# Illumina/manta

Hardware: AMD Instinct MI355X
Metric: candidate SV loci assembled+aligned per second (whole node) (higher is better)
Workload: dtype int32; 1 GPU; BASELINE config[1]: synthetic small-indel loci, 80 reads/locus x150bp, k=31..76 step 5, assemble + 10-mer trim + GlobalLargeIndelAligner(2,-8,-24,-1,-1;-100) on 1800 bp windows; loci_per_gpu=10000, reads_per_locus=80, block_loci=10000, workers_per_gpu=1, parallelism=loci sharded over 1 rank(s); per rank a cost-ordered block queue, queue=rank, dist_world=1, mix=False

## Files before the change

### manta_amd/csrc/asm_contig.hpp

```cpp
#pragma once
#ifdef MANTA_WAVE_EMU
#include <set>
#endif
#include "asm_lds.hpp"

namespace manta_dev {

#ifndef MANTA_CK_FAST_CAP
#define MANTA_CK_FAST_CAP 3
#endif
static const unsigned CK_FAST_CAP = MANTA_CK_FAST_CAP;
static const unsigned CK_MAX_EXT = 1020;

struct CkWsLayout {
  uint64_t lane_seq, lane_bits, lane_meta, lane_log, total;
};
static const unsigned CK_SEQ_WORDS = CK_MAX_EXT / 16 + 2;
static const unsigned CK_LOG_QW    = (CK_MAX_EXT + 4) / 4;
WV_HD CkWsLayout ckWorkspaceLayout(const unsigned setw = 2)
{
  CkWsLayout L;
  uint64_t   o = 0;
  L.lane_seq  = asmPut(o, 64ull * 2 * 4 * CK_SEQ_WORDS);
  L.lane_bits = asmPut(o, 64ull * 2 * setw * 8);
// ... 1037 lines not shown
      for (unsigned q = 0; q < SW; ++q) {
        sup.w[q] = lb[q];
        rej.w[q] = lb[SW + q];
      }
      const int32_t* m   = lane_meta + candSlotV * 8;
      nLeft              = unsigned(m[0]);
      nRight             = unsigned(m[1]);
      consB              = m[2];
      consE              = m[3];
      myLen              = nLeft + k + nRight;
    }
    Set      used = setZero();
    bool     aliveL     = lane < nCand;
    unsigned finalCount = 0;
    uint64_t chosen     = 0;
    uint64_t chosenHi   = 0;
    Set normalS;
    for (unsigned q = 0; q < SW; ++q) {
      const unsigned lo = 64 * q;
      normalS.w[q]      = (nNormal >= lo + 64) ? ~uint64_t(0) : ((nNormal > lo) ? ((uint64_t(1) << (nNormal - lo)) - 1) : uint64_t(0));
    }
    while (finalCount < P.opt.maxAssemblyCount) {
      if (!wv::any(aliveL)) break;
      const unsigned usedNormal = popSet(setAnd(used, normalS));
      if (nNormal - usedNormal < P.opt.minUnusedReads) break;
      const Set      fresh  = setAndNot(sup, used);
      const unsigned nFresh = popSet(fresh);
      if (aliveL && popSet(setAnd(fresh, normalS)) < P.opt.minSupportReads) aliveL = false;
      uint64_t key = aliveL ? ((uint64_t(nFresh) << 40) | (uint64_t(myLen) << 8) | uint64_t(63u - lane)) : 0;
      for (int off = 1; off < 64; off <<= 1) {
        const uint64_t o = wv::shfl(key, wv::lane() ^ off);
        key              = (o > key) ? o : key;
      }
      if ((key >> 40) == 0) break;
      const int selected = wv::first(int(63u - unsigned(key & 63u)));
      if (finalCount < 10)
        chosen |= uint64_t(selected) << (6 * finalCount);
      else
        chosenHi |= uint64_t(selected) << (6 * (finalCount - 10));
      if (int(lane) == selected) aliveL = false;
      for (unsigned q = 0; q < SW; ++q) used.w[q] |= wv::readlane(sup.w[q], selected);
      finalCount++;
    }
    auto chosenAt = [&](const unsigned f) { return unsigned(((f < 10) ? (chosen >> (6 * f)) : (chosenHi >> (6 * (f - 10)))) & 63u); };

    AsmLocusOut out;
    out.status            = ASM_OK;
    out.n_contigs         = finalCount;
    out.n_words           = W;
    const unsigned nP     = st ? wv::first(st->nPseudo) : 0u;
    out.n_pseudo          = nP;
    out.final_word_length = k;
    out.n_iterations      = nIter;
    out.cyclic_iterations = cycIters;
    out.reserved          = 0;
    uint64_t seqBytes = 0;
    for (unsigned f = 0; f < finalCount; ++f) seqBytes += wv::readlane(myLen, int(chosenAt(f)));
    const unsigned pLen = (lane < nP) ? unsigned(st->len[lane]) : 0u;
    {
      unsigned t = pLen;
      for (int off = 1; off < 64; off <<= 1) t += wv::shfl(t, wv::lane() ^ off);
      seqBytes += t;
    }
    const uint64_t     bitsWords = uint64_t(finalCount) * 2 * W + nP;
    unsigned long long seqBase = 0, bitsBase = 0;
    if (lane == 0) {
      seqBase  = wv::atomic_add(P.seq_used, (unsigned long long)seqBytes);
      bitsBase = wv::atomic_add(P.bits_used, (unsigned long long)bitsWords);
    }
    seqBase  = wv::readlane(uint64_t(seqBase), 0);
    bitsBase = wv::readlane(uint64_t(bitsBase), 0);
    if (seqBase + seqBytes > P.seq_cap || bitsBase + bitsWords > P.bits_cap) {
      out.status         = ASM_E_OUT_CAPACITY;
      out.n_contigs      = 0;
      out.pseudo_off     = 0;
      out.pseudo_len_off = 0;
      if (lane == 0) P.loci[locus] = out;
      return;
    }
    uint64_t        so = seqBase, bo = bitsBase;
    const uint16_t* gp = gPb();
    for (unsigned f = 0; f < finalCount; ++f) {
      const int      c   = int(chosenAt(f));
      const unsigned sl  = wv::readlane(candSlotV, c);
      const unsigned nL  = wv::readlane(nLeft, c), nR = wv::readlane(nRight, c), len = nL + k + nR;
      const unsigned seedPb = gp[slotNode[sl]];
      for (unsigned i = lane; i < len; i += 64) P.seq_arena[so + i] = uint8_t("ACGT"[contigCode(sl, nL, seedPb, i)]);
      {
        const unsigned half = lane / W, w = lane % W;
        uint64_t       mine = 0;
        for (unsigned q = 0; q < SW; ++q) {
          const uint64_t sq = wv::readlane(sup.w[q], c), rq = wv::readlane(rej.w[q], c);
          if (w == q) mine = half ? rq : sq;
        }
        if (lane < 2 * W) P.bits_arena[bo + lane] = mine;
      }
      const int cb = wv::readlane(consB, c), ce = wv::readlane(consE, c);
      if (lane == 0) {
        AsmContigOut o;
        o.seq_off    = so;
        o.bits_off   = bo;
        o.seq_len    = len;
        o.cons_begin = cb;
        o.cons_end   = int(len) - ce;
        o.reserved   = 0;
        P.contigs[size_t(locus) * P.opt.maxAssemblyCount + f] = o;
      }
      so += len;
      bo += 2 * W;
    }
    out.pseudo_off     = so;
    out.pseudo_len_off = bo;
    if (nP) {
      const uint32_t* pc = G.parena + st->off;
      unsigned        cw = 0;
      for (unsigned p = 0; p < nP; ++p) {
        const unsigned len = wv::readlane(pLen, int(p));
        for (unsigned i = lane; i < len; i += 64) P.seq_arena[so + i] = uint8_t("ACGT"[(pc[cw + (i >> 4)] >> (30 - 2 * (i & 15))) & 3u]);
        if (lane == 0) P.bits_arena[bo + p] = len;
        so += len;
        cw += (len + 15) / 16 + 1;
      }
    }
    if (lane == 0) P.loci[locus] = out;
    if (!C::BIG && G.sched && shareBytes) scheduleEpilogue(locus, seqBase, finalCount, myLen, chosen, chosenHi);
  }

  WV_DEV void scheduleEpilogue(const unsigned locus, const uint64_t seqBase, const unsigned finalCount, const unsigned myLen, const uint64_t chosen,
                               const uint64_t chosenHi)
  {
    const ScheduleParams& S = *G.sched;
    auto lenAt = [&](const unsigned f) { return wv::readlane(myLen, int(((f < 10) ? (chosen >> (6 * f)) : (chosenHi >> (6 * (f - 10)))) & 63u)); };
    if (shareBytes <= SCHED_TABLE_BYTES + 16) return;
    const unsigned lseqBytes = (shareBytes - SCHED_TABLE_BYTES) & ~15u;
    const uint64_t ro0 = wv::readlane(uint64_t(S.ref_off[locus]), 0), ro1 = wv::readlane(uint64_t(S.ref_off[locus + 1]), 0);
    if (ro1 < ro0 || ro1 - ro0 > lseqBytes) return;
    const unsigned refSize = unsigned(ro1 - ro0);
    bool           fits    = true;
    for (unsigned f = 0; f < finalCount; ++f) {
      const unsigned len = lenAt(f);
      if (!schedTableFitsLds(len) || schedStagedBytes(len, refSize) > lseqBytes) fits = false;
    }
    if (!fits) return;
    wv::sync();
    uint32_t* const ltable = reinterpret_cast<uint32_t*>(lds);
    uint8_t* const  lseq   = reinterpret_cast<uint8_t*>(lds) + SCHED_TABLE_BYTES;
    const unsigned  maxAsm = S.max_assembly_count, total = S.n_loci * maxAsm;
    if (lane >= finalCount && lane < maxAsm) {
      SmallSvTaskInfo none = {0, 0, 0, -1};
      S.info[locus * maxAsm + lane] = none;
    }
    uint64_t so  = seqBase;
    unsigned cig = 0;
    for (unsigned f = 0; f < finalCount; ++f) {
      const unsigned        len  = lenAt(f);
      const unsigned        slot = locus * maxAsm + f;
      const SmallSvTaskInfo info = scheduleContig<false>(S, slot, locus, so, len, ltable, lseq, lseqBytes, nullptr);
      wv::sync();
      const int bucket = wv::first(info.bucket);
      if (lane == 0) {
        S.info[slot] = info;
        if (bucket >= 0) {
          const unsigned b       = unsigned(bucket);
          const unsigned winLen  = refSize - unsigned(info.adj_leading_cut) - unsigned(info.adj_trailing_cut);
          const unsigned slabLen = schedSlabLen(S, b, len, winLen);
          S.bucket_ids[size_t(b) * total + wv::atomic_add(&S.bucket_count[b], 1u)] = slot;
          if (wv::atomic_load(&S.bucket_maxref[b]) < slabLen) wv::atomic_max(&S.bucket_maxref[b], slabLen);
        }
      }
      if (bucket >= 0) cig += 4 * len + 16;
      so += len;
      wv::sync();
    }
    if (lane == 0) {
      S.marks[locus] = 1;
      wv::atomic_add(S.n_marked, 1ull);
      if (cig) wv::atomic_add(S.cigar_used, (unsigned long long)cig);
    }
  }

  WV_DEV int run(const unsigned locus)
  {
    tMark = wv::clock();
#ifdef MANTA_WAVE_EMU
#define CK_TRACE(why) do { if (std::getenv("MANTA_EMU_PUNT_TRACE") && lane == 0) std::fprintf(stderr, "  contig_kernel punts locus %u: %s (%u words, %u with a set, k %u)\n", locus, why, nNodes, nFat, k); } while (0)
#else
#define CK_TRACE(why) do { } while (0)
#endif
    if (!load(locus)) {
      CK_TRACE("does not fit this launch's LDS");
      if (C::BIG && lane == 0 && G.stats) wv::atomic_add(&G.stats[7], 1u);
      return CK_PUNT;
    }
    tick(4);
    if (!acyclic && !cyclic && graphHasCycle()) {
      CK_TRACE("cyclic graph");
      return CK_PUNT;
    }
    tick(3);
    loadPool();
    tick(4);
    anyRep = false;
    if ((C::BIG ? contigRoundsStretch() : contigRounds()) != 0) {
      CK_TRACE("contig too long");
      if (C::BIG && lane == 0 && G.stats) wv::atomic_add(&G.stats[7], 1u);
      return CK_PUNT;
    }
    const bool rounds = C::BIG && G.iter != nullptr;
    if (anyRep && !rounds) {
      CK_TRACE("repeat hit");
      return CK_PUNT;
    }
    const unsigned round    = rounds ? G.round : 0u;
    const unsigned nIter    = round + 1;
    const unsigned cycIters = ((round > 0) ? wv::first(G.iter[locus].cyclicIters) : 0u) + (cyclic ? 1u : 0u);
    const LgIter*  st       = (round > 0) ? &G.iter[locus] : nullptr;
    if (anyRep) {
      if (!writePseudo(locus)) {
        CK_TRACE("pseudo arena full");
        if (lane == 0 && G.stats) wv::atomic_add(&G.stats[8], 1u);
        return CK_PUNT;
      }
      st                   = &G.iter[locus];
      const unsigned maxWL = P.locus_max_wl ? P.locus_max_wl[locus] : P.opt.maxWordLength;
      if (k + P.opt.wordStepSize <= maxWL) {
        if (round >= G.last_round) {
          CK_TRACE("more word lengths than rounds");
          if (lane == 0 && G.stats) wv::atomic_add(&G.stats[9], 1u);
          return CK_PUNT;
        }
        if (lane == 0) {
          LgIter* w      = &G.iter[locus];
          w->k           = k + P.opt.wordStepSize;
          w->nIter       = nIter;
          w->cyclicIters = cycIters;
          G.next_ids[wv::atomic_add(G.next_count, 1u)] = locus;
        }
        LG_STAT(7, 1);
        return CK_NEXT;
      }
    }
    selectAndEmit(locus, st, nIter, cycIters);
    tick(7);
    LG_STAT(0, 1);
    LG_STAT(3, nCand);
    LG_STAT(6, acyclic ? 1u : 0u);
    return CK_DONE;
  }
};

template <class C>
WV_DEV void contigKernelBody(const LgArgs& A)
{
  const AsmParams& P = A.P;
  const LgParams&  G = A.G;
  uint8_t*        ws    = G.cws + uint64_t(wv::block_single()) * G.cws_stride;
  char*           lds   = wv::lds_single();
  const unsigned  nLoci = wv::first(wv::atomic_load(&G.class_count[G.cls]));
  const uint32_t* ids   = G.class_ids + size_t(G.cls) * G.class_stride;
  while (true) {
    unsigned slot = 0;
    if (wv::lane() == 0) slot = wv::atomic_add(P.counter, 1u);
    slot = wv::first(slot);
    if (slot >= nLoci) break;
    const unsigned locus = ids[slot];
    LdsContig<C>   c(P, G, lds, ws);
    c.shareBytes = P.lds_bytes;
    const int      rc = c.run(locus);
    wv::sync();
    if (rc == CK_PUNT && wv::lane() == 0) P.punt_ids[wv::atomic_add(P.punt_count, 1u)] = locus;
    wv::sync();
  }
}
#if !MANTA_TU_DEFINES(MANTA_TU_CONTIG)
WV_KERNEL_SINGLE WV_WAVES_PER_SIMD(2) void contig_kernel(const LgArgs A);
#else
WV_KERNEL_SINGLE WV_WAVES_PER_SIMD(2) void contig_kernel(const LgArgs A)
{
  contigKernelBody<LgS>(A);
}
#endif

static const unsigned CK_POOL_WAVES = 12;
static const unsigned CK_POOL_BYTES = 163840;
static const unsigned CK_POOL_HDR   = 64;
static_assert(4 * (1 + CK_POOL_WAVES) <= CK_POOL_HDR && (CK_POOL_BYTES - CK_POOL_HDR) / 16 < 65536, "pool header");

WV_DEV unsigned ckPoolTake(char* pool, const unsigned w, const unsigned units, uint32_t* stat)
{
  uint32_t*      lock  = reinterpret_cast<uint32_t*>(pool);
  uint32_t*      share = lock + 1;
  const unsigned lane  = unsigned(wv::lane());
  const unsigned capU  = (CK_POOL_BYTES - CK_POOL_HDR) / 16;
  unsigned       polls = 0;
  while (true) {
    ++polls;
    unsigned got = 0;
    if (lane == 0) got = (wv::atomic_cas(lock, 0u, 1u) == 0u) ? 1u : 0u;
    if (wv::first(got)) {
      wv::fence_wg();
      unsigned s = 0;
      if (lane >= 1 && lane <= CK_POOL_WAVES) s = wv::atomic_load(&share[lane - 1]) >> 16;
      bool ok = lane <= CK_POOL_WAVES && s + units <= capU;
      for (unsigned v = 0; v < CK_POOL_WAVES; ++v) {
        const unsigned e = wv::atomic_load(&share[v]), a = e & 0xffffu, b = e >> 16;
        if (a < b && s < b && a < s + units) ok = false;
      }
      const uint64_t m  = wv::ballot(ok);
      const unsigned at = m ? wv::readlane(s, wv::ctz(m)) : 0u;
      if (m && lane == 0) wv::atomic_store(&share[w], at | ((at + units) << 16));
// ... 91 lines not shown
```

### manta_amd/csrc/pipeline_kernels.hpp

```cpp
#pragma once
#include "align_kernels.hpp"
#include "assemble_kernels.hpp"
#include "smallsv_trim.hpp"

namespace manta_dev {

WV_DEV SmallSvTaskInfo scheduleSlot(const ScheduleParams& P, const unsigned slot, uint32_t* ltable, uint32_t* gtable)
{
  const unsigned    locus = slot / P.max_assembly_count, ci = slot % P.max_assembly_count;
  const AsmLocusOut lo    = P.loci[locus];
  if (lo.status != ASM_OK || ci >= lo.n_contigs) {
    SmallSvTaskInfo none = {(lo.status != ASM_OK) ? 1 : 0, 0, 0, -1};
    return none;
  }
  const AsmContigOut co = P.contigs[slot];
  return scheduleContig<true>(P, slot, locus, co.seq_off, co.seq_len, ltable, reinterpret_cast<uint8_t*>(ltable) + SCHED_TABLE_BYTES, SCHED_SEQ_BYTES, gtable);
}

static const unsigned SCHED_PEND = 8;
struct SchedPending {
  uint32_t count[16];
  uint32_t maxref[16];
  uint32_t slot[16][SCHED_PEND];
  uint32_t cigarWords;
};
WV_DEV void schedFlush(const ScheduleParams& P, SchedPending* pend, const unsigned bucket, const unsigned total)
{
  const unsigned n = pend->count[bucket];
  if (n == 0) return;
  unsigned pos = 0;
  if (wv::lane() == 0) {
    pos = wv::atomic_add(&P.bucket_count[bucket], n);
    unsigned cur = wv::atomic_load(&P.bucket_maxref[bucket]);
    const unsigned want = pend->maxref[bucket];
    while (cur < want) {
      const unsigned old = wv::atomic_cas(&P.bucket_maxref[bucket], cur, want);
      if (old == cur) break;
      cur = old;
    }
  }
  pos = wv::first(pos);
  if (unsigned(wv::lane()) < n) P.bucket_ids[size_t(bucket) * total + pos + unsigned(wv::lane())] = pend->slot[bucket][wv::lane()];
  wv::sync();
  if (wv::lane() == 0) {
    pend->count[bucket]  = 0;
    pend->maxref[bucket] = 0;
  }
  wv::sync();
}

#if !MANTA_TU_DEFINES(MANTA_TU_GLUE)
WV_KERNEL void smallsv_schedule_kernel(const ScheduleParams P);
#else
WV_KERNEL void smallsv_schedule_kernel(const ScheduleParams P)
{
  const unsigned lane   = unsigned(wv::lane());
  uint32_t*      gtable = P.table_ws + size_t(wv::block()) * P.table_cap;
  uint32_t*      ltable = reinterpret_cast<uint32_t*>(wv::lds(SCHED_LDS_BYTES));
  SchedPending*  pend   = reinterpret_cast<SchedPending*>(reinterpret_cast<char*>(ltable) + SCHED_TABLE_BYTES + SCHED_SEQ_BYTES);
  const unsigned total  = P.n_loci * P.max_assembly_count;
  if (lane < 16) {
    pend->count[lane]  = 0;
    pend->maxref[lane] = 0;
  }
  if (lane == 0) pend->cigarWords = 0;
  wv::sync();
  while (true) {
    unsigned base = 0;
    if (lane == 0) base = wv::atomic_add(P.counter, P.chunk);
    base = wv::first(base);
    if (base >= P.n_loci) break;
    const unsigned end = (base + P.chunk < P.n_loci) ? base + P.chunk : P.n_loci;
    for (unsigned b0 = base; b0 < end; b0 += 64) {
      uint64_t todo = wv::ballot(b0 + lane < end && !(P.marks && P.marks[b0 + lane]));
      while (todo) {
        const unsigned locus = b0 + unsigned(wv::ctz(todo));
        todo &= todo - 1;
        const AsmLocusOut lo       = P.loci[locus];
        const unsigned    nContigs = (lo.status == ASM_OK) ? lo.n_contigs : 0u;
        if (lane >= nContigs && lane < P.max_assembly_count) {
          SmallSvTaskInfo none = {(lo.status != ASM_OK) ? 1 : 0, 0, 0, -1};
          P.info[locus * P.max_assembly_count + lane] = none;
        }
        for (unsigned ci = 0; ci < nContigs; ++ci) {
          const unsigned        slot = locus * P.max_assembly_count + ci;
          const SmallSvTaskInfo info = scheduleSlot(P, slot, ltable, gtable);
          wv::sync();
          if (lane == 0) P.info[slot] = info;
          if (info.bucket >= 0) {
            const unsigned b = unsigned(info.bucket);
            if (lane == 0) {
              const AlignTaskDev& t = P.tasks[slot];
              const unsigned slabLen = schedSlabLen(P, b, t.query_len, t.ref1_len);
              pend->slot[b][pend->count[b]] = slot;
              pend->count[b] += 1;
              pend->cigarWords += 4 * t.query_len + 16;
              if (slabLen > pend->maxref[b]) pend->maxref[b] = slabLen;
            }
            wv::sync();
            if (pend->count[b] == SCHED_PEND) schedFlush(P, pend, b, total);
          }
          wv::sync();
        }
      }
    }
  }
  for (unsigned b = 0; b < P.n_e; ++b) schedFlush(P, pend, b, total);
  if (lane == 0 && pend->cigarWords) wv::atomic_add(P.cigar_used, (unsigned long long)pend->cigarWords);
}
#endif

static const unsigned BS_CLASSES = 512;
static const unsigned BS_WAVES   = 16;
static const unsigned BS_LDS_BYTES = 4 * (BS_WAVES * BS_CLASSES + BS_CLASSES + 8);
struct BucketSortParams {
  const AlignTaskDev*    tasks;
  const AsmLocusOut*     loci;
  const SmallSvTaskInfo* info;
  uint32_t*              ids_out;
  uint32_t               n_loci, max_assembly_count;
  uint32_t               total;
  uint32_t               mask;
};
#if !MANTA_TU_DEFINES(MANTA_TU_GLUE)
WV_KERNEL_WG(16) void bucket_sort_kernel(const BucketSortParams P);
#else
WV_KERNEL_WG(16) void bucket_sort_kernel(const BucketSortParams P)
{
  const unsigned b = unsigned(wv::block_single());
  if (!((P.mask >> b) & 1u)) return;
  uint32_t*      hist  = reinterpret_cast<uint32_t*>(wv::lds_single());
  uint32_t*      dbase = hist + BS_WAVES * BS_CLASSES;
  const unsigned tw = unsigned(wv::wave_in_wg()), tn = unsigned(wv::wg_waves()), lane = unsigned(wv::lane());
  const unsigned tid = 64 * tw + lane, nt = 64 * tn;
  uint32_t*      out    = P.ids_out + size_t(b) * P.total;
  uint32_t*      myHist = hist + BS_CLASSES * tw;
  const unsigned chunk  = (((P.n_loci + tn - 1) / tn) + 63) & ~63u;
  const unsigned c0 = chunk * tw, c1 = (c0 + chunk < P.n_loci) ? (c0 + chunk) : P.n_loci;
  auto cls = [&](const unsigned id) {
    const unsigned c = P.tasks[id].ref1_len >> 3;
    return (BS_CLASSES - 1) - ((c < BS_CLASSES - 1) ? c : (BS_CLASSES - 1));
  };
  auto contigsOf = [&](const unsigned locus) -> unsigned {
    if (locus >= c1) return 0u;
    const AsmLocusOut lo = P.loci[locus];
    return (lo.status == ASM_OK) ? lo.n_contigs : 0u;
  };
  for (unsigned i = tid; i < BS_WAVES * BS_CLASSES + BS_CLASSES; i += nt) hist[i] = 0;
  wv::sync();
  wv::wg_barrier();
  for (unsigned i0 = c0; i0 < c1; i0 += 64) {
    const unsigned locus = i0 + lane, n = contigsOf(locus);
    for (unsigned ci = 0; ci < n; ++ci) {
      const unsigned slot = locus * P.max_assembly_count + ci;
      if (P.info[slot].bucket == int(b)) wv::atomic_add(&myHist[cls(slot)], 1u);
    }
  }
  wv::sync();
  wv::wg_barrier();
  for (unsigned d = tid; d < BS_CLASSES; d += nt) {
    unsigned run = 0;
    for (unsigned w = 0; w < BS_WAVES; ++w) {
      const unsigned c          = (w < tn) ? hist[BS_CLASSES * w + d] : 0u;
      hist[BS_CLASSES * w + d] = run;
      run += c;
    }
    dbase[d] = run;
  }
  wv::sync();
  wv::wg_barrier();
  if (tw == 0) {
    unsigned v[8], sum = 0;
    for (int j = 0; j < 8; ++j) {
      v[j] = dbase[8 * lane + j];
      sum += v[j];
    }
    unsigned inc = sum;
    for (int off = 1; off < 64; off <<= 1) {
      const unsigned o = wv::shfl(inc, int(lane) - off);
      if (int(lane) >= off) inc += o;
    }
    unsigned run = inc - sum;
    for (int j = 0; j < 8; ++j) {
      dbase[8 * lane + j] = run;
      run += v[j];
    }
  }
  wv::sync();
  wv::wg_barrier();
  for (unsigned i0 = c0; i0 < c1; i0 += 64) {
    const unsigned locus = i0 + lane, n = contigsOf(locus);
    unsigned       nMax  = n;
    for (int off = 32; off > 0; off >>= 1) {
      const unsigned o = wv::shfl(nMax, int(lane) ^ off);
      nMax             = (o > nMax) ? o : nMax;
    }
    for (unsigned ci = 0; ci < nMax; ++ci) {
      const unsigned slot  = locus * P.max_assembly_count + ci;
      const bool     valid = ci < n && P.info[slot].bucket == int(b);
      const unsigned d     = valid ? cls(slot) : 0u;
      uint64_t       peers = wv::ballot(valid);
      for (int bit = 0; bit < 9; ++bit) {
        const bool     on = (d >> bit) & 1u;
        const uint64_t m  = wv::ballot(valid && on);
        peers &= on ? m : ~m;
      }
      unsigned base = 0;
      if (valid) base = dbase[d] + myHist[d];
      wv::sync();
      if (valid) {
        out[base + unsigned(wv::popc(peers & ((uint64_t(1) << lane) - 1)))] = slot;
        if ((peers >> lane) == 1u) myHist[d] += unsigned(wv::popc(peers));
      }
      wv::sync();
    }
  }
}
#endif

struct JumpCuts {
  int32_t a1Lead, a1Trail, a2Lead, a2Trail;
};

struct SpanTaskInfo {
  int32_t status;
  int32_t bucket;
  int32_t bucket2;
  int32_t is_uncut;
};

struct SpanParams {
  const AsmLocusOut*  loci;
  const AsmContigOut* contigs;
  const uint8_t*      seq_arena;
  uint32_t            n_loci, max_assembly_count;
  const uint8_t*      refs1;
  const uint64_t*     ref1_off;
  const uint8_t*      refs2;
  const uint64_t*     ref2_off;
// ... 269 lines not shown
```

### manta_amd/csrc/smallsv_trim.hpp

```cpp
#pragma once
#include "align_kernels.hpp"
#include "assemble_kernels.hpp"

namespace manta_dev {

static const int      SMALLSV_MER       = 10;
static const unsigned SCHED_TABLE_BYTES = 4096;
static const unsigned SCHED_SEQ_BYTES   = 6144;
static const unsigned SCHED_LDS_BYTES   = SCHED_TABLE_BYTES + SCHED_SEQ_BYTES + 1024;

struct SmallSvCuts {
  int32_t leadingCut, trailingCut, maxLeadingCut, maxTrailingCut;
};

struct SmallSvTaskInfo {
  int32_t status;
  int32_t adj_leading_cut, adj_trailing_cut;
  int32_t bucket;
};

struct ScheduleParams {
  const AsmLocusOut*  loci;
  const AsmContigOut* contigs;
  const uint8_t*      seq_arena;
  uint32_t            n_loci;
  uint32_t            max_assembly_count;
  const uint8_t*     refs;
  const uint64_t*    ref_off;
  const SmallSvCuts* cuts;
  AlignTaskDev*    tasks;
  SmallSvTaskInfo* info;
  uint32_t*        bucket_ids;
  uint32_t*        bucket_count;
  uint32_t*        bucket_maxref;
  unsigned long long* cigar_used;
  uint64_t         cigar_cap;
  uint32_t*        counter;
  uint32_t* table_ws;
  uint32_t  table_cap;
  uint64_t e_pack[2];
  uint32_t n_e;
  uint32_t chunk;
  uint8_t*            marks;
  unsigned long long* n_marked;
};

WV_DEV unsigned merCode(const uint8_t* p, bool& valid)
{
  unsigned code = 0;
  valid         = true;
  for (int i = 0; i < SMALLSV_MER; ++i) {
    const unsigned c = baseCode(p[i]);
    if (c > 3) valid = false;
    code = (code << 2) | (c & 3u);
  }
  return code;
}

static const int MER_BATCH = 55;
WV_DEV unsigned merLoadBase(const uint8_t* seq, const int len, const int p0)
{
  const int pos = p0 + wv::lane();
  return (pos >= 0 && pos < len) ? baseCode(seq[pos]) : 4u;
}
WV_DEV unsigned merCodesFromBase(const unsigned c, bool& valid)
{
  const int      l   = wv::lane();
  unsigned bad = (c > 3) ? 1u : 0u;
  unsigned w1  = c & 3u;
  const unsigned w2 = (w1 << 2) | wv::shfl(w1, (l + 1) & 63);
  const unsigned b2 = bad | wv::shfl(bad, (l + 1) & 63);
  const unsigned w4 = (w2 << 4) | wv::shfl(w2, (l + 2) & 63);
  const unsigned b4 = b2 | wv::shfl(b2, (l + 2) & 63);
  const unsigned w8 = (w4 << 8) | wv::shfl(w4, (l + 4) & 63);
  const unsigned b8 = b4 | wv::shfl(b4, (l + 4) & 63);
  const unsigned w10 = (w8 << 4) | wv::shfl(w2, (l + 8) & 63);
  const unsigned b10 = b8 | wv::shfl(b2, (l + 8) & 63);
  valid = (l < MER_BATCH) && (b10 == 0);
  return w10;
}
WV_DEV unsigned merCodes55(const uint8_t* seq, const int len, const int p0, bool& valid)
{
  return merCodesFromBase(merLoadBase(seq, len, p0), valid);
}

WV_DEV bool merLookup(const uint32_t* table, const unsigned mask, const unsigned code)
{
  unsigned s = (code * 2654435761u) & mask;
  while (true) {
    const uint32_t v = table[s];
    if (v == 0) return false;
    if (v == code + 1) return true;
    s = (s + 1) & mask;
  }
}

WV_DEV unsigned merHashBytes(const uint8_t* p)
{
  unsigned h = 2166136261u;
  for (int i = 0; i < SMALLSV_MER; ++i) h = (h ^ p[i]) * 16777619u;
  return h ^ (h >> 15);
}
WV_DEV bool merEqualBytes(const uint8_t* a, const uint8_t* b)
{
  bool eq = true;
  for (int i = 0; i < SMALLSV_MER; ++i) eq = eq && (a[i] == b[i]);
  return eq;
}
WV_DEV bool merLookupBytes(const uint32_t* table, const unsigned mask, const uint8_t* contig, const uint8_t* mer)
{
  unsigned s = merHashBytes(mer) & mask;
  while (true) {
    const uint32_t v = table[s];
    if (v == 0) return false;
    if (merEqualBytes(contig + (v - 1), mer)) return true;
    s = (s + 1) & mask;
  }
}

WV_DEV unsigned schedE(const ScheduleParams& P, const unsigned b)
{
  return unsigned(((b < 8) ? P.e_pack[0] : P.e_pack[1]) >> (8 * (b & 7))) & 255u;
}
WV_HD void schedPackE(ScheduleParams& P, const int* eSet, const unsigned n)
{
  P.n_e       = (n < 16) ? n : 16;
  P.e_pack[0] = P.e_pack[1] = 0;
  for (unsigned b = 0; b < P.n_e; ++b) P.e_pack[b >> 3] |= uint64_t(unsigned(eSet[b]) & 255u) << (8 * (b & 7));
}

WV_HD unsigned schedStagedBytes(const unsigned clen, const unsigned refSize)
{
  return ((clen + 30) & ~15u) + ((refSize + 30) & ~15u);
}
WV_HD bool schedTableFitsLds(const unsigned clen)
{
  return 8 * clen <= SCHED_TABLE_BYTES;
}

template <bool BYTES>
WV_DEV SmallSvTaskInfo scheduleContig(const ScheduleParams& P, const unsigned slot, const unsigned locus, const uint64_t seqOff, const unsigned clen,
                                      uint32_t* ltable, uint8_t* lseq, const unsigned lseqBytes, uint32_t* gtable)
{
  const unsigned     lane    = unsigned(wv::lane());
  SmallSvTaskInfo    info    = {0, 0, 0, -1};
  const uint8_t*     contigG = P.seq_arena + seqOff;
  const uint8_t*     refG    = P.refs + P.ref_off[locus];
  const int          refSize = int(P.ref_off[locus + 1] - P.ref_off[locus]);
  const SmallSvCuts  cuts    = P.cuts[locus];
  const uint8_t* contig = contigG;
  const uint8_t* ref    = refG;
  {
    const uintptr_t gc = reinterpret_cast<uintptr_t>(contigG), gr = reinterpret_cast<uintptr_t>(refG);
    const unsigned  leadC = unsigned(gc & 15), leadR = unsigned(gr & 15);
    const unsigned  bytesC = (leadC + clen + 15) & ~15u, bytesR = (leadR + unsigned(refSize > 0 ? refSize : 0) + 15) & ~15u;
    if (bytesC + bytesR <= lseqBytes) {
      const u32x4* sc = reinterpret_cast<const u32x4*>(gc - leadC);
      const u32x4* sr = reinterpret_cast<const u32x4*>(gr - leadR);
      u32x4*       dc = reinterpret_cast<u32x4*>(lseq);
      u32x4*       dr = reinterpret_cast<u32x4*>(lseq + bytesC);
      for (unsigned i = lane; i < bytesC / 16; i += 64) dc[i] = sc[i];
      for (unsigned i = lane; i < bytesR / 16; i += 64) dr[i] = sr[i];
      wv::sync();
      contig = lseq + leadC;
      ref    = lseq + bytesC + leadR;
    }
  }

  if (clen < unsigned(SMALLSV_MER) || 2 * clen > P.table_cap) {
    info.status = 2;
    return info;
  }
  unsigned tcap = 64;
  while (tcap < 2 * clen) tcap <<= 1;
  const unsigned mask  = tcap - 1;
  uint32_t*      table = (tcap * 4 <= SCHED_TABLE_BYTES) ? ltable : gtable;
  for (unsigned i = lane; i < tcap; i += 64) table[i] = 0;
  bool exact = false;
  if (BYTES) {
    bool other = false;
    for (unsigned i = lane; i < clen; i += 64) other = other || (baseCode(contig[i]) > 3);
    exact = wv::any(other);
  }
  wv::sync();
  if (BYTES && exact) {
    for (unsigned p = lane; p + SMALLSV_MER <= clen; p += 64) {
      unsigned s = merHashBytes(contig + p) & mask;
      while (true) {
        const uint32_t old = wv::atomic_cas(&table[s], 0u, p + 1);
        if (old == 0 || merEqualBytes(contig + (old - 1), contig + p)) break;
        s = (s + 1) & mask;
      }
    }
  }
  for (int p0 = 0; !exact && p0 + SMALLSV_MER <= int(clen); p0 += MER_BATCH) {
    bool           valid;
    const unsigned code = merCodes55(contig, int(clen), p0, valid);
    if (!valid) continue;
    unsigned s = (code * 2654435761u) & mask;
    while (true) {
      const uint32_t old = wv::atomic_cas(&table[s], 0u, code + 1);
      if (old == 0 || old == code + 1) break;
      s = (s + 1) & mask;
    }
  }
  wv::sync();
  if (table == gtable) wv::fence_acquire();

  const int minRefIndex    = cuts.leadingCut;
  const int maxRefIndex    = refSize - (cuts.trailingCut + SMALLSV_MER);
  const int maxFwdRefIndex = (cuts.maxLeadingCut < maxRefIndex) ? cuts.maxLeadingCut : maxRefIndex;
  int adjLead = maxFwdRefIndex + 1;
  if (adjLead < minRefIndex) adjLead = minRefIndex;
  const int minRevRefIndex = (minRefIndex > refSize - cuts.maxTrailingCut) ? minRefIndex : (refSize - cuts.maxTrailingCut);
  int       revIndex       = minRevRefIndex - 1;
  if (revIndex > maxRefIndex) revIndex = maxRefIndex;
  {
    int  fBase = minRefIndex, bTop = maxRefIndex;
    bool fDone = fBase > maxFwdRefIndex, bDone = bTop < minRevRefIndex;
    while (!fDone || !bDone) {
      const int      bBase = bTop - (MER_BATCH - 1);
      const unsigned cf = merLoadBase(ref, refSize, fDone ? -1000 : fBase), cb = merLoadBase(ref, refSize, bDone ? -1000 : bBase);
      bool           vf, vb;
      const unsigned codeF = merCodesFromBase(cf, vf), codeB = merCodesFromBase(cb, vb);
      const int      iF = fBase + int(lane), iB = bBase + int(lane);
      bool           hitF, hitB;
      if (BYTES && exact) {
        const bool inF = lane < unsigned(MER_BATCH) && iF >= 0 && iF + SMALLSV_MER <= refSize;
        const bool inB = lane < unsigned(MER_BATCH) && iB >= 0 && iB + SMALLSV_MER <= refSize;
        hitF = !fDone && inF && iF <= maxFwdRefIndex && merLookupBytes(table, mask, contig, ref + iF);
        hitB = !bDone && inB && iB >= minRevRefIndex && iB <= bTop && merLookupBytes(table, mask, contig, ref + iB);
      } else {
        hitF = !fDone && vf && iF <= maxFwdRefIndex && merLookup(table, mask, codeF);
        hitB = !bDone && vb && iB >= minRevRefIndex && iB <= bTop && merLookup(table, mask, codeB);
      }
      const uint64_t mF = wv::ballot(hitF), mB = wv::ballot(hitB);
      if (!fDone) {
        if (mF) {
          adjLead = fBase + wv::ctz(mF);
          fDone   = true;
        } else {
          fBase += MER_BATCH;
          fDone = fBase > maxFwdRefIndex;
        }
      }
      if (!bDone) {
        if (mB) {
          revIndex = bBase + (63 - wv::clz(mB));
          bDone    = true;
        } else {
          bTop -= MER_BATCH;
          bDone = bTop < minRevRefIndex;
        }
      }
    }
  }
  const int adjTrail = refSize - (revIndex + SMALLSV_MER);
  const int winLen   = refSize - adjLead - adjTrail;
  info.adj_leading_cut  = adjLead;
  info.adj_trailing_cut = adjTrail;
  if (winLen <= 0 || adjLead < 0 || adjTrail < 0) {
    info.status = 3;
    return info;
  }
  int            bucket = -1;
  const unsigned need   = (clen + 63) / 64;
  for (unsigned b = 0; b < P.n_e; ++b)
    if (schedE(P, b) >= need) {
      bucket = int(b);
      break;
    }
  if (bucket < 0) bucket = int(P.n_e) - 1;
  const unsigned long long cig = 8ull * seqOff;
  if (cig + 4ull * clen + 16 > P.cigar_cap) {
    info.status = 5;
    return info;
  }
  if (lane == 0) {
    AlignTaskDev t;
    t.query     = contigG;
    t.ref1      = refG + adjLead;
    t.ref2      = nullptr;
    t.query_len = clen;
    t.ref1_len  = unsigned(winLen);
    t.ref2_len  = 0;
    t.cigar_off = uint32_t(cig);
    P.tasks[slot] = t;
  }
  info.bucket = bucket;
  return info;
}

WV_DEV unsigned schedSlabLen(const ScheduleParams& P, const unsigned bucket, const unsigned clen, const unsigned winLen)
{
  return unsigned(alignSlabRefLen(1, int(schedE(P, bucket)), clen, winLen));
}

}
```

Before: 1.317 million loci/s.

## Stage reference once per locus and scan 10-mers in per-lane 12-wide chunks

Reference window staging into LDS moves out of the per-contig routine into a per-locus scheduleLocus step, so contigs of the same locus reuse the staged reference. The per-lane shuffle-based 55-mer batches are replaced by per-lane chunks of 12 consecutive 10-mers decoded from packed 32-bit words. Each pass therefore covers 768 positions, with batched table inserts and lookups plus a slow-path fallback on collisions. Forward and backward scans now alternate instead of running together, which adds wasted work past the first hit and more register pressure.

Result: slower. 1.253 million loci/s (-4.8%).

```diff
diff --git a/manta_amd/csrc/asm_contig.hpp b/manta_amd/csrc/asm_contig.hpp
--- a/manta_amd/csrc/asm_contig.hpp
+++ b/manta_amd/csrc/asm_contig.hpp
@@ -1213,10 +1213,11 @@
     }
     uint64_t so  = seqBase;
     unsigned cig = 0;
+    const TrimWindow win = scheduleLocus(S, locus, lseq, lseqBytes);
     for (unsigned f = 0; f < finalCount; ++f) {
       const unsigned        len  = lenAt(f);
       const unsigned        slot = locus * maxAsm + f;
-      const SmallSvTaskInfo info = scheduleContig<false>(S, slot, locus, so, len, ltable, lseq, lseqBytes, nullptr);
+      const SmallSvTaskInfo info = scheduleContig<false>(S, slot, win, so, len, ltable, lseq, lseqBytes, nullptr);
       wv::sync();
       const int bucket = wv::first(info.bucket);
       if (lane == 0) {
diff --git a/manta_amd/csrc/pipeline_kernels.hpp b/manta_amd/csrc/pipeline_kernels.hpp
--- a/manta_amd/csrc/pipeline_kernels.hpp
+++ b/manta_amd/csrc/pipeline_kernels.hpp
@@ -5,16 +5,10 @@
 
 namespace manta_dev {
 
-WV_DEV SmallSvTaskInfo scheduleSlot(const ScheduleParams& P, const unsigned slot, uint32_t* ltable, uint32_t* gtable)
-{
-  const unsigned    locus = slot / P.max_assembly_count, ci = slot % P.max_assembly_count;
-  const AsmLocusOut lo    = P.loci[locus];
-  if (lo.status != ASM_OK || ci >= lo.n_contigs) {
-    SmallSvTaskInfo none = {(lo.status != ASM_OK) ? 1 : 0, 0, 0, -1};
-    return none;
-  }
+WV_DEV SmallSvTaskInfo scheduleSlot(const ScheduleParams& P, const unsigned slot, const TrimWindow& W, uint32_t* ltable, uint32_t* gtable)
+{
   const AsmContigOut co = P.contigs[slot];
-  return scheduleContig<true>(P, slot, locus, co.seq_off, co.seq_len, ltable, reinterpret_cast<uint8_t*>(ltable) + SCHED_TABLE_BYTES, SCHED_SEQ_BYTES, gtable);
+  return scheduleContig<true>(P, slot, W, co.seq_off, co.seq_len, ltable, reinterpret_cast<uint8_t*>(ltable) + SCHED_TABLE_BYTES, SCHED_SEQ_BYTES, gtable);
 }
 
 static const unsigned SCHED_PEND = 8;
@@ -82,9 +76,11 @@
           SmallSvTaskInfo none = {(lo.status != ASM_OK) ? 1 : 0, 0, 0, -1};
           P.info[locus * P.max_assembly_count + lane] = none;
         }
+        TrimWindow win = {nullptr, {0, 0, 0, 0}, {nullptr, 0, 0, 0}, 0};
+        if (nContigs) win = scheduleLocus(P, locus, reinterpret_cast<uint8_t*>(ltable) + SCHED_TABLE_BYTES, SCHED_SEQ_BYTES);
         for (unsigned ci = 0; ci < nContigs; ++ci) {
           const unsigned        slot = locus * P.max_assembly_count + ci;
-          const SmallSvTaskInfo info = scheduleSlot(P, slot, ltable, gtable);
+          const SmallSvTaskInfo info = scheduleSlot(P, slot, win, ltable, gtable);
           wv::sync();
           if (lane == 0) P.info[slot] = info;
           if (info.bucket >= 0) {
diff --git a/manta_amd/csrc/smallsv_trim.hpp b/manta_amd/csrc/smallsv_trim.hpp
--- a/manta_amd/csrc/smallsv_trim.hpp
+++ b/manta_amd/csrc/smallsv_trim.hpp
@@ -57,31 +57,67 @@
   return code;
 }
 
-static const int MER_BATCH = 55;
-WV_DEV unsigned merLoadBase(const uint8_t* seq, const int len, const int p0)
-{
-  const int pos = p0 + wv::lane();
-  return (pos >= 0 && pos < len) ? baseCode(seq[pos]) : 4u;
-}
-WV_DEV unsigned merCodesFromBase(const unsigned c, bool& valid)
-{
-  const int      l   = wv::lane();
-  unsigned bad = (c > 3) ? 1u : 0u;
-  unsigned w1  = c & 3u;
-  const unsigned w2 = (w1 << 2) | wv::shfl(w1, (l + 1) & 63);
-  const unsigned b2 = bad | wv::shfl(bad, (l + 1) & 63);
-  const unsigned w4 = (w2 << 4) | wv::shfl(w2, (l + 2) & 63);
-  const unsigned b4 = b2 | wv::shfl(b2, (l + 2) & 63);
-  const unsigned w8 = (w4 << 8) | wv::shfl(w4, (l + 4) & 63);
-  const unsigned b8 = b4 | wv::shfl(b4, (l + 4) & 63);
-  const unsigned w10 = (w8 << 4) | wv::shfl(w2, (l + 8) & 63);
-  const unsigned b10 = b8 | wv::shfl(b2, (l + 8) & 63);
-  valid = (l < MER_BATCH) && (b10 == 0);
-  return w10;
-}
-WV_DEV unsigned merCodes55(const uint8_t* seq, const int len, const int p0, bool& valid)
-{
-  return merCodesFromBase(merLoadBase(seq, len, p0), valid);
+struct TrimText {
+  const uint8_t* units;
+  unsigned       lead;
+  unsigned       bytes;
+  int            len;
+  WV_DEV const uint8_t* text() const { return units + lead; }
+};
+WV_DEV TrimText trimTextAt(const uint8_t* g, const int len)
+{
+  const unsigned lead = unsigned(reinterpret_cast<uintptr_t>(g) & 15);
+  const TrimText t    = {g - lead, lead, (lead + unsigned(len > 0 ? len : 0) + 15) & ~15u, len};
+  return t;
+}
+WV_DEV unsigned trimLane()
+{
+  unsigned l = unsigned(wv::lane());
+#ifndef MANTA_WAVE_EMU
+  asm volatile("" : "+v"(l));
+#endif
+  return l;
+}
+WV_DEV TrimText trimStage(const TrimText& t, uint8_t* dst)
+{
+  const u32x4* s = reinterpret_cast<const u32x4*>(t.units);
+  u32x4*       d = reinterpret_cast<u32x4*>(dst);
+  for (unsigned i = trimLane(); i < t.bytes / 16; i += 64) d[i] = s[i];
+  TrimText r = t;
+  r.units    = dst;
+  return r;
+}
+
+static const int TRIM_CH   = 12;
+static const int TRIM_PASS = 64 * TRIM_CH;
+static const int TRIM_DW   = (TRIM_CH + 9 + 3) / 4;
+WV_DEV int trimPassBase(const TrimText& t, const int i)
+{
+  return i - ((int(t.lead) + i) & 3);
+}
+WV_DEV unsigned trimChunkCodes(const TrimText& t, const int p0, const int lo, const int hi, unsigned (&codes)[TRIM_CH])
+{
+  const uint32_t* u   = reinterpret_cast<const uint32_t*>(t.units);
+  const int       off = int(t.lead) + p0;
+  uint32_t        w[TRIM_DW];
+#pragma unroll
+  for (int j = 0; j < TRIM_DW; ++j) {
+    const unsigned o = unsigned(off + 4 * j);
+    w[j]             = u[((o < t.bytes) ? o : 0u) >> 2];
+  }
+  unsigned code = 0, clear = 0, ok = 0;
+#pragma unroll
+  for (int j = 0; j < TRIM_CH + 9; ++j) {
+    const unsigned c = baseCode(uint8_t(w[j >> 2] >> (8 * (j & 3))));
+    clear            = (c <= 3 && unsigned(p0 + j) < unsigned(t.len)) ? clear + 1 : 0u;
+    code             = ((code << 2) | (c & 3u)) & 0xfffffu;
+    if (j >= 9) {
+      const int q = j - 9, i = p0 + q;
+      codes[q]    = code;
+      if (clear >= unsigned(SMALLSV_MER) && i >= lo && i <= hi) ok |= 1u << q;
+    }
+  }
+  return ok;
 }
 
 WV_DEV bool merLookup(const uint32_t* table, const unsigned mask, const unsigned code)
@@ -139,33 +175,76 @@
 }
 
 template <bool BYTES>
-WV_DEV SmallSvTaskInfo scheduleContig(const ScheduleParams& P, const unsigned slot, const unsigned locus, const uint64_t seqOff, const unsigned clen,
+WV_DEV unsigned trimPassHits(const TrimText& t, const int p0, const int lo, const int hi, const uint32_t* table, const unsigned mask, const bool exact,
+                             const uint8_t* contig)
+{
+  unsigned hits = 0;
+  if (BYTES && exact) {
+    for (int q = 0; q < TRIM_CH; ++q) {
+      const int i = p0 + q;
+      if (i >= lo && i <= hi && i >= 0 && i + SMALLSV_MER <= t.len && merLookupBytes(table, mask, contig, t.text() + i)) hits |= 1u << q;
+    }
+    return hits;
+  }
+  unsigned       codes[TRIM_CH];
+  const unsigned ok   = trimChunkCodes(t, p0, lo, hi, codes);
+  unsigned       more = 0, v[TRIM_CH];
+#pragma unroll
+  for (int q = 0; q < TRIM_CH; ++q) v[q] = table[(codes[q] * 2654435761u) & mask];
+#pragma unroll
+  for (int q = 0; q < TRIM_CH; ++q) {
+    if (v[q] == codes[q] + 1) hits |= 1u << q;
+    if (v[q] != 0) more |= 1u << q;
+  }
+  hits &= ok;
+  more &= ok & ~hits;
+  while (more) {
+    const int q = wv::ctz(uint64_t(more));
+    more &= more - 1;
+    bool valid;
+    if (merLookup(table, mask, merCode(t.text() + p0 + q, valid))) hits |= 1u << q;
+  }
+  return hits;
+}
+
+struct TrimWindow {
+  const uint8_t* refG;
+  SmallSvCuts    cuts;
+  TrimText       ref;
+  unsigned       staged;
+};
+WV_DEV TrimWindow scheduleLocus(const ScheduleParams& P, const unsigned locus, uint8_t* lseq, const unsigned lseqBytes)
+{
+  TrimWindow W;
+  W.refG   = P.refs + P.ref_off[locus];
+  W.cuts   = P.cuts[locus];
+  W.ref    = trimTextAt(W.refG, int(P.ref_off[locus + 1] - P.ref_off[locus]));
+  W.staged = 0;
+  if (W.ref.bytes <= lseqBytes) {
+    W.ref    = trimStage(W.ref, lseq);
+    W.staged = W.ref.bytes;
+    wv::sync();
+  }
+  return W;
+}
+
+template <bool BYTES>
+WV_DEV SmallSvTaskInfo scheduleContig(const ScheduleParams& P, const unsigned slot, const TrimWindow& W, const uint64_t seqOff, const unsigned clen,
                                       uint32_t* ltable, uint8_t* lseq, const unsigned lseqBytes, uint32_t* gtable)
 {
   const unsigned     lane    = unsigned(wv::lane());
   SmallSvTaskInfo    info    = {0, 0, 0, -1};
   const uint8_t*     contigG = P.seq_arena + seqOff;
-  const uint8_t*     refG    = P.refs + P.ref_off[locus];
-  const int          refSize = int(P.ref_off[locus + 1] - P.ref_off[locus]);
-  const SmallSvCuts  cuts    = P.cuts[locus];
-  const uint8_t* contig = contigG;
-  const uint8_t* ref    = refG;
-  {
-    const uintptr_t gc = reinterpret_cast<uintptr_t>(contigG), gr = reinterpret_cast<uintptr_t>(refG);
-    const unsigned  leadC = unsigned(gc & 15), leadR = unsigned(gr & 15);
-    const unsigned  bytesC = (leadC + clen + 15) & ~15u, bytesR = (leadR + unsigned(refSize > 0 ? refSize : 0) + 15) & ~15u;
-    if (bytesC + bytesR <= lseqBytes) {
-      const u32x4* sc = reinterpret_cast<const u32x4*>(gc - leadC);
-      const u32x4* sr = reinterpret_cast<const u32x4*>(gr - leadR);
-      u32x4*       dc = reinterpret_cast<u32x4*>(lseq);
-      u32x4*       dr = reinterpret_cast<u32x4*>(lseq + bytesC);
-      for (unsigned i = lane; i < bytesC / 16; i += 64) dc[i] = sc[i];
-      for (unsigned i = lane; i < bytesR / 16; i += 64) dr[i] = sr[i];
-      wv::sync();
-      contig = lseq + leadC;
-      ref    = lseq + bytesC + leadR;
-    }
-  }
+  const uint8_t*     refG    = W.refG;
+  const int          refSize = W.ref.len;
+  const SmallSvCuts  cuts    = W.cuts;
+  TrimText ctext = trimTextAt(contigG, int(clen));
+  if (ctext.bytes + W.staged <= lseqBytes) {
+    ctext = trimStage(ctext, lseq + W.staged);
+    wv::sync();
+  }
+  const TrimText& rtext  = W.ref;
+  const uint8_t*  contig = ctext.text();
 
   if (clen < unsigned(SMALLSV_MER) || 2 * clen > P.table_cap) {
     info.status = 2;
@@ -193,15 +272,30 @@
       }
     }
   }
-  for (int p0 = 0; !exact && p0 + SMALLSV_MER <= int(clen); p0 += MER_BATCH) {
-    bool           valid;
-    const unsigned code = merCodes55(contig, int(clen), p0, valid);
-    if (!valid) continue;
-    unsigned s = (code * 2654435761u) & mask;
-    while (true) {
-      const uint32_t old = wv::atomic_cas(&table[s], 0u, code + 1);
-      if (old == 0 || old == code + 1) break;
-      s = (s + 1) & mask;
+  for (int base = trimPassBase(ctext, 0); !exact && base + SMALLSV_MER <= int(clen); base += TRIM_PASS) {
+    unsigned       codes[TRIM_CH], old[TRIM_CH];
+    const int      p0 = base + int(trimLane()) * TRIM_CH;
+    const unsigned ok = trimChunkCodes(ctext, p0, 0, int(clen) - SMALLSV_MER, codes);
+#pragma unroll
+    for (int q = 0; q < TRIM_CH; ++q) {
+      old[q] = 0;
+      if ((ok >> q) & 1u) old[q] = wv::atomic_cas(&table[(codes[q] * 2654435761u) & mask], 0u, codes[q] + 1);
+    }
+    unsigned more = 0;
+#pragma unroll
+    for (int q = 0; q < TRIM_CH; ++q)
+      if (old[q] != 0 && old[q] != codes[q] + 1) more |= 1u << q;
+    while (more) {
+      const int q = wv::ctz(uint64_t(more));
+      more &= more - 1;
+      bool           valid;
+      const unsigned code = merCode(contig + p0 + q, valid);
+      unsigned       s    = (code * 2654435761u) & mask;
+      while (true) {
+        s                  = (s + 1) & mask;
+        const uint32_t o   = wv::atomic_cas(&table[s], 0u, code + 1);
+        if (o == 0 || o == code + 1) break;
+      }
     }
   }
   wv::sync();
@@ -216,41 +310,32 @@
   int       revIndex       = minRevRefIndex - 1;
   if (revIndex > maxRefIndex) revIndex = maxRefIndex;
   {
-    int  fBase = minRefIndex, bTop = maxRefIndex;
-    bool fDone = fBase > maxFwdRefIndex, bDone = bTop < minRevRefIndex;
+    const int lastStart = refSize - SMALLSV_MER;
+    const int fLo = (minRefIndex > 0) ? minRefIndex : 0, fHi = (maxFwdRefIndex < lastStart) ? maxFwdRefIndex : lastStart;
+    const int bLo = (minRevRefIndex > 0) ? minRevRefIndex : 0, bHi = (maxRefIndex < lastStart) ? maxRefIndex : lastStart;
+    int       fBase = trimPassBase(rtext, fLo), bTop = bHi;
+    bool      fDone = fLo > fHi, bDone = bLo > bHi;
     while (!fDone || !bDone) {
-      const int      bBase = bTop - (MER_BATCH - 1);
-      const unsigned cf = merLoadBase(ref, refSize, fDone ? -1000 : fBase), cb = merLoadBase(ref, refSize, bDone ? -1000 : bBase);
-      bool           vf, vb;
-      const unsigned codeF = merCodesFromBase(cf, vf), codeB = merCodesFromBase(cb, vb);
-      const int      iF = fBase + int(lane), iB = bBase + int(lane);
-      bool           hitF, hitB;
-      if (BYTES && exact) {
-        const bool inF = lane < unsigned(MER_BATCH) && iF >= 0 && iF + SMALLSV_MER <= refSize;
-        const bool inB = lane < unsigned(MER_BATCH) && iB >= 0 && iB + SMALLSV_MER <= refSize;
-        hitF = !fDone && inF && iF <= maxFwdRefIndex && merLookupBytes(table, mask, contig, ref + iF);
-        hitB = !bDone && inB && iB >= minRevRefIndex && iB <= bTop && merLookupBytes(table, mask, contig, ref + iB);
-      } else {
-        hitF = !fDone && vf && iF <= maxFwdRefIndex && merLookup(table, mask, codeF);
-        hitB = !bDone && vb && iB >= minRevRefIndex && iB <= bTop && merLookup(table, mask, codeB);
-      }
-      const uint64_t mF = wv::ballot(hitF), mB = wv::ballot(hitB);
-      if (!fDone) {
-        if (mF) {
-          adjLead = fBase + wv::ctz(mF);
+      const bool     fwd   = !fDone;
+      const int      bBase = trimPassBase(rtext, bTop - (TRIM_PASS - 4));
+      const int      p0    = (fwd ? fBase : bBase) + int(trimLane()) * TRIM_CH;
+      const unsigned hits  = trimPassHits<BYTES>(rtext, p0, fwd ? fLo : bLo, fwd ? fHi : bTop, table, mask, exact, contig);
+      const uint64_t m     = wv::ballot(hits != 0);
+      if (fwd) {
+        if (m) {
+          adjLead = wv::readlane(p0 + wv::ctz(uint64_t(hits) | (uint64_t(1) << TRIM_CH)), wv::ctz(m));
           fDone   = true;
         } else {
-          fBase += MER_BATCH;
-          fDone = fBase > maxFwdRefIndex;
+          fBase += TRIM_PASS;
+          fDone = fBase > fHi;
         }
-      }
-      if (!bDone) {
-        if (mB) {
-          revIndex = bBase + (63 - wv::clz(mB));
+      } else {
+        if (m) {
+          revIndex = wv::readlane(p0 + 63 - wv::clz(uint64_t(hits) | 1u), 63 - wv::clz(m));
           bDone    = true;
         } else {
-          bTop -= MER_BATCH;
-          bDone = bTop < minRevRefIndex;
+          bTop  = bBase - 1;
+          bDone = bTop < bLo;
         }
       }
     }
```
